# kepengxu/RealCamNet

Hardware: AMD Instinct MI355X
Metric: megapixels/sec RAW->sRGB at 4K (higher is better)
Workload: dtype bf16; 1 GPU; cfg3: 3840x2160 Bayer mosaic -> unshuffle+pad16 -> LiteISPNet_GFM_LSC_GMA -> sRGB 3840x2160, 8 frames/GPU, bf16 storage / fp32 accumulate; frames_per_gpu=8, global_frames=8, parallelism=frame-shard x1, collective=none

## Files before the change

realcamnet_amd/csrc/conv.hip:

```cpp
#include <mutex>
#include <vector>

#include "conv32_kernel.hpp"

namespace rc {

struct ConvPlan {
    int ck = 0, nt = 0, unit = 0, upt = 0, nu = 0, steps = 0;
    int n_chunks = 0, n_ct = 0, cout_packed = 0;
    int m32 = 0;
};

static int g_persist_on = 1;
extern int g_dw3_seg16;
extern int g_dec_lds;
extern int g_wmsa_mfma;
extern int g_pw_grid_cap;
static int g_pss = 0;
static int g_poison = 0;
static int g_thin = 2;
static int g_auto = 1;
static int g_sums_compact = 1;
static int g_conv32 = 0;

static bool make_plan(int cin, int cout, int ksize, int dtype, int out_mode, ConvPlan* p, int cout_tile = 0) {
    if (cin < 1 || cout < 1 || (ksize != 1 && ksize != 3 && ksize != 2 && ksize != 5)) return false;
    if (dtype != RC_F32 && dtype != RC_BF16 && dtype != RC_F16) return false;
    const bool h16 = dtype != RC_F32;
    if (ksize == 5 && (cout > 16 || out_mode == RC_OUT_PIXEL_SHUFFLE2 || (h16 ? (cin % 48 != 0 && cin % 32 != 0) : cin % 16 != 0))) return false;
    if (out_mode == RC_OUT_PIXEL_SHUFFLE2_NCHW && cout % 4 != 0) return false;
    if (ksize == 2 && (dtype != RC_BF16 || cin % 16 != 0 || out_mode != RC_OUT_NHWC || (cin % 48 == 0 && cin % 64 != 0))) return false;
    p->unit = dtype == RC_F32 ? 4 : 8;
    if (ksize == 5) p->ck = h16 ? (cin % 48 == 0 ? 48 : 32) : 16;
    else if (h16) {
        if (cin <= 8) p->ck = 8;
        else if (ksize == 1 && cin % 80 == 0 && cin % 64 != 0) p->ck = 80;
        else if (ksize >= 2 && cin % 64 == 0 && cin > 64) p->ck = 32;
        else if (cin % 64 == 0) p->ck = 64;
        else if (cin % 48 == 0) p->ck = 48;
        else if (ksize == 3 && cin == 32) p->ck = 32;
        else if (ksize == 3 && cin % 32 == 0 && cin > 64) p->ck = 32;
        else p->ck = 16;
    } else {
        p->ck = cin <= 4 ? 4 : 16;
    }
    if (out_mode == RC_OUT_PIXEL_SHUFFLE2) {
        if (cout % 4 != 0) return false;
        const int cps = cout / 4;
        if (cps % 64 == 0 && !(cps % 48 == 0 && h16 && cin == 48)) p->nt = 4;
        else if (cps % 48 == 0) p->nt = 3;
        else if (cps % 64 == 0) p->nt = 4;
        else if (cps % 16 == 0) p->nt = 1;
        else return false;
    } else if (cout % 48 == 0 && h16 && cin == 48) p->nt = 3;
    else if (h16 && ksize == 3 && cin == 32 && cout == 32) p->nt = 2;
    else if (ksize == 1 && cout % 80 == 0) p->nt = 5;
    else if (cout % 64 == 0) p->nt = 4;
    else if (cout % 48 == 0) p->nt = 3;
    else if (h16 && ksize == 3 && p->ck == 32 && cout % 32 == 0) p->nt = 2;
    else p->nt = 1;
    if (cout_tile != 0) {
        if (cout_tile < 16 || cout_tile > 80 || cout_tile % 16 != 0 || ksize == 5 || ksize == 2 || out_mode == RC_OUT_PIXEL_SHUFFLE2 || out_mode == RC_OUT_PIXEL_SHUFFLE2_NCHW) return false;
        p->nt = cout_tile / 16;
    }
    p->m32 = 0;
    if (cout_tile == 0 && dtype == RC_BF16 && ksize == 3 && g_conv32 != 0 && cout <= kPersistMaxCout && out_mode != RC_OUT_NCHW && out_mode != RC_OUT_PIXEL_SHUFFLE2_NCHW) {
        const int cw = out_mode == RC_OUT_PIXEL_SHUFFLE2 ? cout / 4 : cout;
        const bool all = g_conv32 != 4;
        if (all && p->ck == 32 && cin % 32 == 0 && (out_mode == RC_OUT_PIXEL_SHUFFLE2 ? cw % 32 == 0 : cw % 64 == 0)) { p->m32 = 1; p->nt = 2; p->ck = (g_conv32 == 1 && out_mode == RC_OUT_NHWC) ? 16 : 32; }
        else if (cin == 48 && (out_mode == RC_OUT_PIXEL_SHUFFLE2 ? (all && cw % 48 == 0) : cw % 96 == 0)) { p->m32 = 1; p->nt = 3; p->ck = 48; }
// ... 147 lines not shown
        const int co = packed_to_cout(p, cout, out_mode, j);
        dst[j] = (bias && co >= 0 && co < cout) ? bias[co] : 0.f;
    }
    return RC_OK;
}

size_t rc_conv_desc_size(void) { return sizeof(rc_conv_desc); }

int rc_tail_fold_weights(const float* w1, const float* b1, const float* w2, const float* b2, int c, int o, float* wc, float* bc) {
    RC_REQUIRE(w1 && w2 && wc && bc && c >= 1 && o >= 1, "rc_tail_fold_weights: bad arguments");
    std::vector<double> acc((size_t)4 * o * c * 25, 0.0), bacc((size_t)4 * o, 0.0);
    for (int oo = 0; oo < o; ++oo)
        for (int i = 0; i < 2; ++i)
            for (int j = 0; j < 2; ++j) {
                const int row = oo * 4 + 2 * i + j;
                bacc[row] = b2 ? (double)b2[oo] : 0.0;
                for (int dy = 0; dy < 3; ++dy)
                    for (int dx = 0; dx < 3; ++dx) {
                        const int a = i + dy - 1, b = j + dx - 1;
                        const int fy = a < 0 ? -1 : a >> 1, ii = a & 1, fx = b < 0 ? -1 : b >> 1, jj = b & 1;
                        for (int cc = 0; cc < c; ++cc) {
                            const int m = 4 * cc + 2 * ii + jj;
                            const double v2 = w2[(((size_t)oo * c + cc) * 3 + dy) * 3 + dx];
                            if (b1) bacc[row] += v2 * (double)b1[m];
                            for (int k = 0; k < c; ++k)
                                for (int ey = 0; ey < 3; ++ey)
                                    for (int ex = 0; ex < 3; ++ex)
                                        acc[(((size_t)row * c + k) * 5 + (fy + ey + 1)) * 5 + (fx + ex + 1)] += v2 * (double)w1[(((size_t)m * c + k) * 3 + ey) * 3 + ex];
                        }
                    }
            }
    for (size_t n = 0; n < acc.size(); ++n) wc[n] = (float)acc[n];
    for (size_t n = 0; n < bacc.size(); ++n) bc[n] = (float)bacc[n];
    return RC_OK;
}

int rc_conv_sum_tiles(int height, int width) { return 4 * ceil_div(height, kTH) * ceil_div(width, kTW); }

int rc_debug_set(const char* key, int value) {
    RC_REQUIRE(key != nullptr, "rc_debug_set: null key");
    if (std::string(key) == "persist") { g_persist_on = value < 0 ? 0 : (value > 3 ? 3 : value); return RC_OK; }
    if (std::string(key) == "conv_flags") { g_dbg_flags = value; return RC_OK; }
    if (std::string(key) == "pair_impl") { g_pair_impl = value < 0 || value > 2 ? 0 : value; return RC_OK; }
    if (std::string(key) == "dec_lds") { g_dec_lds = value != 0; return RC_OK; }
    if (std::string(key) == "dw3_seg16") { g_dw3_seg16 = value != 0; return RC_OK; }
    if (std::string(key) == "wmsa_mfma") { g_wmsa_mfma = value != 0; return RC_OK; }
    if (std::string(key) == "pss") { g_pss = value != 0; return RC_OK; }
    if (std::string(key) == "sums_compact") { g_sums_compact = value != 0; return RC_OK; }
    if (std::string(key) == "persist_auto") { g_auto = value < 0 ? 0 : (value > 2 ? 2 : value); return RC_OK; }
    if (std::string(key) == "thin") { g_thin = value < 0 ? 0 : (value > 2 ? 2 : value); return RC_OK; }
    if (std::string(key) == "lds_poison") { g_poison = value != 0; return RC_OK; }
    if (std::string(key) == "conv32") { g_conv32 = value < 0 ? 0 : (value > 4 ? 4 : value); return RC_OK; }
    if (std::string(key) == "wino_nnt") { wino_set_nnt(value); return RC_OK; }
    if (std::string(key) == "pw_grid_cap") { g_pw_grid_cap = value <= 0 || value > (1 << 22) ? (1 << 22) : value; return RC_OK; }
    return fail(RC_ERR_INVALID, std::string("rc_debug_set: unknown key ") + key);
}

int rc_debug_get(const char* key) {
    if (key == nullptr) return -1;
    if (std::string(key) == "persist") return g_persist_on;
    if (std::string(key) == "conv32") return g_conv32;
    if (std::string(key) == "conv_flags") return g_dbg_flags;
    if (std::string(key) == "pss") return g_pss;
    if (std::string(key) == "sums_compact") return g_sums_compact;
    if (std::string(key) == "persist_auto") return g_auto;
    if (std::string(key) == "thin") return g_thin;
    if (std::string(key) == "lds_poison") return g_poison;
    if (std::string(key) == "wino_nnt") return wino_get_nnt();
    if (std::string(key) == "pw_grid_cap") return g_pw_grid_cap;
    return -1;
}

int rc_debug_set_ptr(const char* key, void* p) {
    RC_REQUIRE(key != nullptr, "rc_debug_set_ptr: null key");
    if (std::string(key) == "conv_phase_timing") { g_dbg_ptr = static_cast<long long*>(p); return RC_OK; }
    return fail(RC_ERR_INVALID, std::string("rc_debug_set_ptr: unknown key ") + key);
}

int rc_prof_enable(int on) {
    std::lock_guard<std::mutex> lk(g_prof_mu);
    for (auto& r : g_prof) { (void)hipEventDestroy(r.e0); (void)hipEventDestroy(r.e1); }
    g_prof.clear();
    g_prof_on = on != 0;
    return RC_OK;
}

int rc_prof_collect(int64_t* n_launches, double* total_ms, double* total_flops) {
    std::lock_guard<std::mutex> lk(g_prof_mu);
    double ms = 0.0, fl = 0.0;
    for (auto& r : g_prof) {
        RC_HIP_CHECK(hipEventSynchronize(r.e1));
        float t = 0.f;
        RC_HIP_CHECK(hipEventElapsedTime(&t, r.e0, r.e1));
        ms += t; fl += r.flops;
    }
    if (n_launches) *n_launches = (int64_t)g_prof.size();
    if (total_ms) *total_ms = ms;
    if (total_flops) *total_flops = fl;
    return RC_OK;
}

int rc_prof_collect_rows(rc_prof_row* rows, int max_rows, int* n_rows) {
    RC_REQUIRE(rows != nullptr && n_rows != nullptr && max_rows >= 1, "rc_prof_collect_rows: bad arguments");
    std::lock_guard<std::mutex> lk(g_prof_mu);
    int n = 0;
    for (auto& r : g_prof) {
        RC_HIP_CHECK(hipEventSynchronize(r.e1));
        float t = 0.f;
        RC_HIP_CHECK(hipEventElapsedTime(&t, r.e0, r.e1));
        int i = 0;
        while (i < n && !(rows[i].cin == r.cin && rows[i].cout == r.cout && rows[i].ksize == r.ksize)) ++i;
        if (i == n) {
            if (n == max_rows) continue;
            rows[n] = rc_prof_row{r.cin, r.cout, r.ksize, 0, 0.0, 0.0, 0.0};
            ++n;
        }
        rows[i].launches += 1; rows[i].ms += t; rows[i].flops += r.flops; rows[i].bytes += r.bytes;
    }
    *n_rows = n;
    return RC_OK;
}

static int conv_build_args(const rc_conv_desc* d, ConvPlan& p, ConvArgs& a, size_t& es_out) {
    RC_REQUIRE(d != nullptr, "rc_conv2d: null desc");
    const bool dwt = d->out_mode == RC_OUT_NHWC_DWT;
    RC_REQUIRE(make_plan(d->cin, d->cout, d->ksize, d->dtype, dwt ? (int)RC_OUT_NHWC : d->out_mode, &p, d->cout_tile), "rc_conv2d: unsupported cin/cout/ksize/dtype/cout_tile");
    RC_REQUIRE(d->batch >= 1 && d->height >= 1 && d->width >= 1, "rc_conv2d: empty tensor");
    RC_REQUIRE(d->batch <= 65535, "rc_conv2d: batch > 65535");
// ... 153 lines not shown
```

realcamnet_amd/csrc/gma_fused.hip:

```cpp
#include "common.hpp"

namespace rc {
namespace gf {

typedef short s16x4 __attribute__((ext_vector_type(4)));

constexpr int kNT = 4;
constexpr int kC = 80, kCT = 64, kSEG = 16, kHID = 320;

__host__ __device__ constexpr int tile_bytes(int cin) { return (cin / 32) * 1024 + ((cin % 32) ? 512 : 0); }
__host__ __device__ constexpr int n_mtiles(int cout) { return (cout + 15) / 16; }
__host__ __device__ constexpr int row_channel(int m, int R, int mt) {
    return (m < (mt & ~1)) ? 32 * (m >> 1) + 8 * (R >> 2) + 4 * (m & 1) + (R & 3) : 16 * m + R;
}

template <int C> struct Act {
    static constexpr int KS = C / 32;
    static constexpr bool TAIL = (C % 32) != 0;
    uint4 f[KS > 0 ? KS : 1];
    uint2 t;
};

__device__ __forceinline__ void mma32(const uint4& a, const uint4& b, f32x4& c) {
    c = __builtin_amdgcn_mfma_f32_16x16x32_bf16(__builtin_bit_cast(bf16x8, a), __builtin_bit_cast(bf16x8, b), c, 0, 0, 0);
// ... 1382 lines not shown
    }
}
#undef GI_KEEP

}
}

extern "C" int rc_dw_toeplitz_pack(const float* taps, int K, int n_ch, void* dst) {
    using namespace rc;
    RC_REQUIRE(taps && dst, "rc_dw_toeplitz_pack: null pointer");
    RC_REQUIRE((K == 3 || K == 5 || K == 7) && n_ch >= 1, "rc_dw_toeplitz_pack: K = 3, 5 or 7");
    uint16_t* out = static_cast<uint16_t*>(dst);
    for (int dy = 0; dy < K; ++dy)
        for (int c = 0; c < n_ch; ++c)
            for (int lane = 0; lane < 64; ++lane)
                for (int i = 0; i < 8; ++i) {
                    const int ox = lane & 15, slot = 8 * (lane >> 4) + i, dx = slot - 4 - ox + K / 2;
                    out[((size_t)(dy * n_ch + c) * 64 + lane) * 8 + i] = (dx >= 0 && dx < K) ? host_f32_to_bf16(taps[(size_t)(dy * K + dx) * n_ch + c]) : (uint16_t)0;
                }
    return RC_OK;
}

extern "C" int rc_gma_in_cpe(const void* d_d1, const void* d_w_in_natural, const float* d_b_in, const void* d_toeplitz3, const float* d_b_cpe, void* d_x,
                             int batch, int H, int W, void* stream) {
    using namespace rc;
    using namespace rc::gf;
    RC_REQUIRE(d_d1 && d_w_in_natural && d_toeplitz3 && d_x, "rc_gma_in_cpe: null pointer");
    RC_REQUIRE(reinterpret_cast<uintptr_t>(d_d1) % 16 == 0 && reinterpret_cast<uintptr_t>(d_w_in_natural) % 16 == 0 && reinterpret_cast<uintptr_t>(d_toeplitz3) % 16 == 0 &&
               reinterpret_cast<uintptr_t>(d_x) % 16 == 0, "rc_gma_in_cpe: misaligned tensor");
    RC_REQUIRE(batch >= 1 && H >= 1 && W >= 1, "rc_gma_in_cpe: bad shape");
    RC_REQUIRE((long long)H * W * GI_CIN * 2 < (1ll << 31), "rc_gma_in_cpe: a 192-channel image must stay below 2 GiB (32-bit buffer offsets)");
    GiArgs a;
    a.d1 = static_cast<const bf16_t*>(d_d1); a.x = static_cast<bf16_t*>(d_x);
    a.batch = batch; a.H = H; a.W = W; a.tiles_x = ceil_div(W, GI_TW); a.tiles_y = ceil_div(H, GI_TH);
    const long long n_tiles = (long long)a.tiles_x * a.tiles_y * batch;
    RC_REQUIRE(n_tiles < (1ll << 31), "rc_gma_in_cpe: too many tiles");
    a.n_tiles = (int)n_tiles;
    a.w_in = d_w_in_natural; a.b_in = d_b_in; a.toep = static_cast<const char*>(d_toeplitz3); a.b_cpe = d_b_cpe;
    const int num_cus = device_cu_count();
    if (int e_ = allow_lds<&gma_in_cpe_kernel>(160 * 1024)) return e_;
    int blocks = a.n_tiles < num_cus ? a.n_tiles : num_cus;
    a.tiles_per_block = (a.n_tiles + blocks - 1) / blocks;
    blocks = (a.n_tiles + a.tiles_per_block - 1) / a.tiles_per_block;
    return launch_lds<&gma_in_cpe_kernel>(dim3((unsigned)blocks), dim3(GI_THREADS), GI_LDS, as_stream(stream), a);
}

namespace rc {
namespace gf {

struct LscArgs {
    const bf16_t* x; int cin0;
    const char* blob; int n_mid; float slope;
    const bf16_t* raw; int raw_c;
    bf16_t* out; long long pixels; int H, W;
};

template <int C> __host__ __device__ constexpr int lsc_weight_bytes(int n_mid, bool head) {
    return (C / 16) * 512 + n_mid * (C / 16) * tile_bytes(C) + (head ? (C / 16) * 1536 : 0);
}

template <int CIN, int MT>
__device__ __forceinline__ void gemm_fresh(const char* w, int lane, const Act<CIN> (&in)[kNT], f32x4 (&acc)[MT][kNT], const float* bias = nullptr, int g = 0) {
    constexpr int KS = CIN / 32, TB = tile_bytes(CIN);
    const f32x4 z = f32x4{0.f, 0.f, 0.f, 0.f};
    if (bias != nullptr) {
#pragma unroll
        for (int m = 0; m < MT; ++m) {
            const f32x4 b = bias4(bias, m, g);
#pragma unroll
            for (int nt = 0; nt < kNT; ++nt) acc[m][nt] = b;
        }
    }
#pragma unroll
    for (int s = 0; s < KS; ++s) {
        uint4 a[MT];
#pragma unroll
        for (int m = 0; m < MT; ++m) a[m] = *reinterpret_cast<const uint4*>(w + m * TB + s * 1024 + lane * 16);
#pragma unroll
        for (int m = 0; m < MT; ++m)
#pragma unroll
            for (int nt = 0; nt < kNT; ++nt) {
                if (s == 0 && bias == nullptr) { acc[m][nt] = z; }
                mma32(a[m], in[nt].f[s], acc[m][nt]);
            }
    }
    if constexpr ((CIN % 32) != 0) {
#pragma unroll
        for (int m = 0; m < MT; ++m) {
            const uint2 a = *reinterpret_cast<const uint2*>(w + m * TB + KS * 1024 + lane * 8);
#pragma unroll
            for (int nt = 0; nt < kNT; ++nt) {
                if (KS == 0 && bias == nullptr) { acc[m][nt] = z; }
                mma16(a, in[nt].t, acc[m][nt]);
            }
        }
    }
}

__device__ __forceinline__ f32x4 leaky4(const f32x4& v, float slope) {
    const f32x4 s = v * slope;
    const float inf = 3.402823466e+38f;
    return f32x4{__builtin_amdgcn_fmed3f(v[0], s[0], inf), __builtin_amdgcn_fmed3f(v[1], s[1], inf), __builtin_amdgcn_fmed3f(v[2], s[2], inf), __builtin_amdgcn_fmed3f(v[3], s[3], inf)};
}

template <int C, bool ACT, bool BIASED = false>
__device__ __forceinline__ void lsc_pack(const f32x4 (&acc)[C / 16][kNT], const float* bias, int g, float slope, Act<C> (&out)[kNT]) {
    constexpr int MT = C / 16;
    auto fin = [&](const f32x4& v, const f32x4& b) {
        f32x4 r = BIASED ? v : v + b;
        if constexpr (ACT) r = leaky4(r, slope);
        return r;
    };
    constexpr bool RAW_ACC = BIASED && !ACT;
#pragma unroll
    for (int p = 0; p < MT / 2; ++p) {
        const f32x4 b0 = bias4(bias, 2 * p, g), b1 = bias4(bias, 2 * p + 1, g);
#pragma unroll
        for (int nt = 0; nt < kNT; ++nt) {
            if constexpr (RAW_ACC) {
                const uint2 lo = qa_pack(acc[2 * p][nt]), hi = qa_pack(acc[2 * p + 1][nt]);
                out[nt].f[p] = make_uint4(lo.x, lo.y, hi.x, hi.y);
            } else {
                out[nt].f[p] = pack_pair(fin(acc[2 * p][nt], b0), fin(acc[2 * p + 1][nt], b1));
            }
        }
    }
    if constexpr (MT & 1) {
        const f32x4 b0 = bias4(bias, MT - 1, g);
#pragma unroll
        for (int nt = 0; nt < kNT; ++nt) {
            if constexpr (RAW_ACC) out[nt].t = qa_pack(acc[MT - 1][nt]);
            else out[nt].t = pack_tail(fin(acc[MT - 1][nt], b0));
        }
    }
}

constexpr int kOOBoff = (int)0x80000000;

struct LscIn {
    uint2 x[kNT];
    uint4 rf[kNT]; uint2 rt[kNT];
};

template <bool HEAD>
__device__ __forceinline__ void lsc_load(const LscArgs& a, long long p0, int n, int g, __amdgpu_buffer_rsrc_t r_x, __amdgpu_buffer_rsrc_t r_raw, LscIn& in) {
    const unsigned uW = (unsigned)a.W, uH = (unsigned)a.H;
    unsigned row0 = 0, x0 = 0, y0 = 0;
    if constexpr (HEAD) {
        row0 = __builtin_amdgcn_readfirstlane((unsigned)p0 / uW);
        x0 = (unsigned)p0 - row0 * uW;
        y0 = __builtin_amdgcn_readfirstlane(row0 % uH);
    }
#pragma unroll
    for (int nt = 0; nt < kNT; ++nt) {
        const long long p = p0 + 16 * nt + n;
        const bool live = p < a.pixels;
        {
            const int off = (live && g == 0) ? (int)p * a.cin0 * 2 : kOOBoff;
            unsigned lo = 0, hi = 0;
            if (a.cin0 == 2) lo = __builtin_amdgcn_raw_buffer_load_b32(r_x, off, 0, 0);
            else if (a.cin0 == 4) { const auto v = __builtin_amdgcn_raw_buffer_load_b64(r_x, off, 0, 0); lo = v[0]; hi = v[1]; }
            else {
                unsigned short e[4] = {0, 0, 0, 0};
                for (int i = 0; i < a.cin0; ++i) e[i] = __builtin_amdgcn_raw_buffer_load_b16(r_x, off == kOOBoff ? kOOBoff : off + 2 * i, 0, 0);
                lo = e[0] | ((unsigned)e[1] << 16); hi = e[2] | ((unsigned)e[3] << 16);
            }
            in.x[nt] = make_uint2(lo, hi);
        }
        if constexpr (HEAD) {
            unsigned x = x0 + 16 * nt + n, y = y0;
            while (x >= uW) { x -= uW; ++y; }
            while (y >= uH) y -= uH;
            auto tap = [&](int t) -> uint2 {
                const int dy = t / 3 - 1, dx = t % 3 - 1;
                const bool ok = live && (unsigned)((int)y + dy) < uH && (unsigned)((int)x + dx) < uW;
                const int off = ok ? ((int)p + dy * a.W + dx) * a.raw_c * 2 : kOOBoff;
                if (a.raw_c == 4) { const auto v = __builtin_amdgcn_raw_buffer_load_b64(r_raw, off, 0, 0); return make_uint2(v[0], v[1]); }
                unsigned short e[4] = {0, 0, 0, 0};
                for (int i = 0; i < a.raw_c; ++i) e[i] = __builtin_amdgcn_raw_buffer_load_b16(r_raw, ok ? off + 2 * i : kOOBoff, 0, 0);
                return make_uint2(e[0] | ((unsigned)e[1] << 16), e[2] | ((unsigned)e[3] << 16));
            };
            const uint2 t0 = tap(2 * g), t1 = tap(2 * g + 1), t8 = tap(8);
            in.rf[nt] = make_uint4(t0.x, t0.y, t1.x, t1.y);
            in.rt[nt] = g == 0 ? t8 : make_uint2(0u, 0u);
        }
    }
}

struct LscTaps { int dy0, dx0, dy1, dx1, d0, d1, d8; };
__device__ __forceinline__ LscTaps lsc_taps(int g, int W) {
    LscTaps t;
    t.dy0 = (2 * g) / 3 - 1; t.dx0 = (2 * g) % 3 - 1; t.dy1 = (2 * g + 1) / 3 - 1; t.dx1 = (2 * g + 1) % 3 - 1;
    t.d0 = (t.dy0 * W + t.dx0) * 8; t.d1 = (t.dy1 * W + t.dx1) * 8; t.d8 = (W + 1) * 8;
    return t;
}
template <bool HEAD>
__device__ __forceinline__ void lsc_load_fast(const LscArgs& a, int p0, unsigned tx0, unsigned ty0, int n, int g, const LscTaps& tp, __amdgpu_buffer_rsrc_t r_x,
                                              __amdgpu_buffer_rsrc_t r_raw, LscIn& in) {
    const unsigned uW = (unsigned)a.W, uH = (unsigned)a.H;
    const int npix = (int)a.pixels;
#pragma unroll
    for (int nt = 0; nt < kNT; ++nt) {
        const int p = p0 + 16 * nt + n;
        const bool live = p < npix;
        in.x[nt] = make_uint2(__builtin_amdgcn_raw_buffer_load_b32(r_x, (live && g == 0) ? p * 4 : kOOBoff, 0, 0), 0u);
        if constexpr (HEAD) {
            unsigned x = tx0 + 16 * nt + n, y = ty0;
            const bool wrap = x >= uW;
            x = wrap ? x - uW : x; y = wrap ? y + 1 : y; y = y == uH ? 0u : y;
            const int pb = p * 8;
            const bool ok0 = live && (unsigned)((int)y + tp.dy0) < uH && (unsigned)((int)x + tp.dx0) < uW;
            const bool ok1 = live && (unsigned)((int)y + tp.dy1) < uH && (unsigned)((int)x + tp.dx1) < uW;
            const bool ok8 = live && g == 0 && y + 1 < uH && x + 1 < uW;
            const auto t0 = __builtin_amdgcn_raw_buffer_load_b64(r_raw, ok0 ? pb + tp.d0 : kOOBoff, 0, 0);
            const auto t1 = __builtin_amdgcn_raw_buffer_load_b64(r_raw, ok1 ? pb + tp.d1 : kOOBoff, 0, 0);
            const auto t8 = __builtin_amdgcn_raw_buffer_load_b64(r_raw, ok8 ? pb + tp.d8 : kOOBoff, 0, 0);
            in.rf[nt] = make_uint4(t0[0], t0[1], t1[0], t1[1]);
            in.rt[nt] = make_uint2(t8[0], t8[1]);
        }
    }
}

template <int C> constexpr int lsc_threads() { return C > 64 ? 512 : 256; }
template <int C, bool HEAD>
__global__ __launch_bounds__(lsc_threads<C>(), 2) void lsc_chain_kernel(const LscArgs a) {
    constexpr int kLscThreads = lsc_threads<C>();
    constexpr int MT = C / 16, TBM = tile_bytes(C);
    extern __shared__ __attribute__((aligned(16))) char lds[];
    const int tid = threadIdx.x, lane = tid & 63, n = lane & 15, g = lane >> 4;
    const int w_bytes = lsc_weight_bytes<C>(a.n_mid, HEAD);
    const int total = w_bytes + (1 + a.n_mid + (HEAD ? 1 : 0)) * MT * 16 * 4;
    for (int i = tid; i < total / 16; i += kLscThreads) reinterpret_cast<uint4*>(lds)[i] = reinterpret_cast<const uint4*>(a.blob)[i];
    __syncthreads();
    constexpr bool STAGE = C <= 64;
    [[maybe_unused]] char* s_stage = lds + ((total + 15) & ~15);
    const char* s_l0 = lds;
    const char* s_mid = lds + MT * 512;
    const char* s_head = s_mid + a.n_mid * MT * TBM;
    const float* s_b = reinterpret_cast<const float*>(lds + w_bytes);

    const __amdgpu_buffer_rsrc_t r_x = __builtin_amdgcn_make_buffer_rsrc(const_cast<bf16_t*>(a.x), 0, (int)(a.pixels * a.cin0 * 2), 0x00020000);
    const __amdgpu_buffer_rsrc_t r_raw = __builtin_amdgcn_make_buffer_rsrc(const_cast<bf16_t*>(HEAD ? a.raw : a.x), 0,
                                                                           (int)(a.pixels * (HEAD ? a.raw_c : a.cin0) * 2), 0x00020000);
    const long long n_tiles = (a.pixels + 63) / 64, n_waves = (long long)gridDim.x * (kLscThreads / 64);
    long long tile = (long long)blockIdx.x * (kLscThreads / 64) + __builtin_amdgcn_readfirstlane(tid >> 6);
    const bool fast = a.cin0 == 2 && (!HEAD || a.raw_c == 4) && a.W >= 64;
    const LscTaps tp = lsc_taps(g, a.W);
    const unsigned uW = (unsigned)a.W, uH = (unsigned)a.H;
    const unsigned step = (unsigned)(64 * n_waves), sx = step % uW, sy = (step / uW) % uH;
    unsigned tx0 = 0, ty0 = 0;
    if (tile < n_tiles) { const unsigned p0 = (unsigned)(tile * 64), row0 = p0 / uW; tx0 = p0 - row0 * uW; ty0 = row0 % uH; }
    auto load = [&](long long t, LscIn& dst) {
        if (fast) {
            lsc_load_fast<HEAD>(a, (int)(t * 64), tx0, ty0, n, g, tp, r_x, r_raw, dst);
            tx0 += sx; ty0 += sy;
            if (tx0 >= uW) { tx0 -= uW; ++ty0; }
            if (ty0 >= uH) ty0 -= uH;
        } else {
            lsc_load<HEAD>(a, t * 64, n, g, r_x, r_raw, dst);
        }
    };
    LscIn nxt;
    if (tile < n_tiles) load(tile, nxt);
    for (; tile < n_tiles; tile += n_waves) {
        const LscIn in = nxt;
        if (tile + n_waves < n_tiles) load(tile + n_waves, nxt);
        Act<C> cur[kNT];
        {
            auto leaky = [&](f32x4 v) { return leaky4(v, a.slope); };
#pragma unroll
            for (int p = 0; p < MT / 2; ++p) {
                const uint2 w0 = *reinterpret_cast<const uint2*>(s_l0 + (2 * p) * 512 + lane * 8), w1 = *reinterpret_cast<const uint2*>(s_l0 + (2 * p + 1) * 512 + lane * 8);
                const f32x4 b0 = bias4(s_b, 2 * p, g), b1 = bias4(s_b, 2 * p + 1, g);
#pragma unroll
                for (int nt = 0; nt < kNT; ++nt) {
                    f32x4 a0 = b0, a1 = b1;
                    mma16(w0, in.x[nt], a0); mma16(w1, in.x[nt], a1);
                    cur[nt].f[p] = pack_pair(leaky(a0), leaky(a1));
                }
            }
            if constexpr (MT & 1) {
                const uint2 w0 = *reinterpret_cast<const uint2*>(s_l0 + (MT - 1) * 512 + lane * 8);
                const f32x4 b0 = bias4(s_b, MT - 1, g);
#pragma unroll
                for (int nt = 0; nt < kNT; ++nt) {
                    f32x4 a0 = b0;
                    mma16(w0, in.x[nt], a0);
                    cur[nt].t = pack_tail(leaky(a0));
                }
            }
        }
#pragma unroll 1
        for (int l = 0; l < a.n_mid; ++l) {
            if constexpr (MT <= 4) {
                f32x4 acc[MT][kNT];
                gemm_fresh<C, MT>(s_mid + l * MT * TBM, lane, cur, acc, s_b + (1 + l) * MT * 16, g);
                if (l + 1 < a.n_mid) lsc_pack<C, true, true>(acc, s_b + (1 + l) * MT * 16, g, a.slope, cur);
                else lsc_pack<C, false, true>(acc, s_b + (1 + l) * MT * 16, g, a.slope, cur);
            } else {
                static_assert(MT % 4 == 0, "wide chain: whole groups of 4 output tiles");
                Act<C> nxt[kNT];
#pragma unroll
                for (int h = 0; h < MT / 4; ++h) {
                    f32x4 acc[4][kNT];
                    const float* bias = s_b + (1 + l) * MT * 16 + 4 * h * 16;
                    gemm_fresh<C, 4>(s_mid + (l * MT + 4 * h) * TBM, lane, cur, acc, bias, g);
                    const bool act = l + 1 < a.n_mid;
#pragma unroll
                    for (int p = 0; p < 2; ++p) {
#pragma unroll
                        for (int nt = 0; nt < kNT; ++nt) {
                            f32x4 v0 = acc[2 * p][nt], v1 = acc[2 * p + 1][nt];
                            if (act) {
                                nxt[nt].f[2 * h + p] = pack_pair(leaky4(v0, a.slope), leaky4(v1, a.slope));
                            } else {
                                const uint2 lo = qa_pack(v0), hi = qa_pack(v1);
                                nxt[nt].f[2 * h + p] = make_uint4(lo.x, lo.y, hi.x, hi.y);
                            }
                        }
                    }
                }
#pragma unroll
                for (int nt = 0; nt < kNT; ++nt) cur[nt] = nxt[nt];
            }
        }
        if constexpr (HEAD) {
            const float* hb = s_b + (1 + a.n_mid) * MT * 16;
            auto head_tile = [&](int m, int nt, const f32x4& b) {
                f32x4 acc = b;
                mma32(*reinterpret_cast<const uint4*>(s_head + m * 1536 + lane * 16), in.rf[nt], acc);
                mma16(*reinterpret_cast<const uint2*>(s_head + m * 1536 + 1024 + lane * 8), in.rt[nt], acc);
                return acc;
            };
            auto mulp1 = [](const f32x4& h, const f32x4& l) { return __builtin_elementwise_fma(h, l, h); };
#pragma unroll
            for (int p = 0; p < MT / 2; ++p) {
                const f32x4 b0 = bias4(hb, 2 * p, g), b1 = bias4(hb, 2 * p + 1, g);
#pragma unroll
                for (int nt = 0; nt < kNT; ++nt)
                    cur[nt].f[p] = pack_pair(mulp1(head_tile(2 * p, nt, b0), up_lo(cur[nt].f[p])), mulp1(head_tile(2 * p + 1, nt, b1), up_hi(cur[nt].f[p])));
            }
            if constexpr (MT & 1) {
                const f32x4 b0 = bias4(hb, MT - 1, g);
#pragma unroll
                for (int nt = 0; nt < kNT; ++nt) cur[nt].t = pack_tail(mulp1(head_tile(MT - 1, nt, b0), up_tail(cur[nt].t)));
            }
        }
        if constexpr (STAGE) {
            char* st = s_stage + (tid >> 6) * (64 * C * 2);
#pragma unroll
            for (int nt = 0; nt < kNT; ++nt) store_act<C>(reinterpret_cast<bf16_t*>(st) + (16 * nt + n) * C, g, cur[nt]);
            __builtin_amdgcn_fence(__ATOMIC_RELEASE, "wavefront");
            __builtin_amdgcn_wave_barrier();
            const long long left = (a.pixels - tile * 64) * (C * 2);
            const __amdgpu_buffer_rsrc_t r_o = __builtin_amdgcn_make_buffer_rsrc(a.out + tile * 64 * C, 0, (int)(left < 64 * C * 2 ? left : 64 * C * 2), 0x00020000);
#pragma unroll
            for (int j = 0; j < (64 * C * 2) / 1024; ++j) {
                const uint4 v = *reinterpret_cast<const uint4*>(st + (lane + 64 * j) * 16);
                typedef unsigned int u4_t __attribute__((ext_vector_type(4)));
                __builtin_amdgcn_raw_buffer_store_b128(u4_t{v.x, v.y, v.z, v.w}, r_o, (lane + 64 * j) * 16, 0, 0);
            }
        } else {
#pragma unroll
            for (int nt = 0; nt < kNT; ++nt) {
                const long long p = tile * 64 + 16 * nt + n;
                if (p < a.pixels) store_act<C>(a.out + p * C, g, cur[nt]);
            }
        }
    }
}

}
}

extern "C" size_t rc_lsc_packed_bytes(int c, int n_mid, int has_head) {
    if (!(c == 32 || c == 48 || c == 64 || c == 128) || n_mid < 1) return 0;
    const bool hd = has_head != 0;
    const int w = c == 32 ? lsc_weight_bytes<32>(n_mid, hd) : c == 48 ? lsc_weight_bytes<48>(n_mid, hd) : c == 64 ? lsc_weight_bytes<64>(n_mid, hd) : lsc_weight_bytes<128>(n_mid, hd);
    return (size_t)w + (size_t)(1 + n_mid + (has_head ? 1 : 0)) * (c / 16) * 16 * 4;
}

extern "C" int rc_lsc_pack(const float* w0, const float* b0, int cin0, const float* const* wmid, const float* const* bmid, int n_mid,
                           const float* whead, const float* bhead, int raw_c, int c, void* dst) {
    RC_REQUIRE(w0 && wmid && bmid && dst, "rc_lsc_pack: null pointer");
    RC_REQUIRE((c == 32 || c == 48 || c == 64 || c == 128) && n_mid >= 1 && n_mid <= 4 && cin0 >= 1 && cin0 <= 4, "rc_lsc_pack: width 32, 48, 64 or 128, 1..4 mid layers, cin0 <= 4");
    RC_REQUIRE(!whead || (raw_c >= 1 && raw_c <= 4), "rc_lsc_pack: the head's input has 1..4 channels");
    const int mt = c / 16, tbm = tile_bytes(c);
    char* p = static_cast<char*>(dst);
    for (int m = 0; m < mt; ++m)
        for (int lane = 0; lane < 64; ++lane) {
            const int ch = row_channel(m, lane & 15, mt), q = lane >> 4;
            uint16_t* o = reinterpret_cast<uint16_t*>(p + m * 512 + lane * 8);
            for (int i = 0; i < 4; ++i) o[i] = (4 * q + i < cin0) ? host_f32_to_bf16(w0[(size_t)ch * cin0 + 4 * q + i]) : 0;
        }
    p += mt * 512;
    for (int l = 0; l < n_mid; ++l) {
        RC_REQUIRE(wmid[l] != nullptr, "rc_lsc_pack: null layer");
        const int rc = rc_chain_pack_weights(wmid[l], c, c, p);
        if (rc != RC_OK) return rc;
        p += mt * tbm;
    }
    if (whead) {
        for (int m = 0; m < mt; ++m)
            for (int lane = 0; lane < 64; ++lane) {
                const int ch = row_channel(m, lane & 15, mt), q = lane >> 4;
                uint16_t* o4 = reinterpret_cast<uint16_t*>(p + m * 1536 + lane * 16);
                uint16_t* o2 = reinterpret_cast<uint16_t*>(p + m * 1536 + 1024 + lane * 8);
                auto wv = [&](int tap, int ci) { return ci < raw_c ? host_f32_to_bf16(whead[((size_t)ch * raw_c + ci) * 9 + tap]) : (uint16_t)0; };
                for (int i = 0; i < 8; ++i) o4[i] = wv(2 * q + (i >> 2), i & 3);
                for (int i = 0; i < 4; ++i) o2[i] = q == 0 ? wv(8, i) : (uint16_t)0;
            }
        p += mt * 1536;
    }
    float* b = reinterpret_cast<float*>(p);
    rc_chain_pack_bias(b0, c, b);
    for (int l = 0; l < n_mid; ++l) rc_chain_pack_bias(bmid[l], c, b + (1 + l) * mt * 16);
    if (whead) rc_chain_pack_bias(bhead, c, b + (1 + n_mid) * mt * 16);
    return RC_OK;
}

extern "C" int rc_lsc_chain(const void* d_x, int cin0, const void* d_blob, int c, int n_mid, float slope, const void* d_raw, int raw_c,
                            void* d_out, int batch, int H, int W, void* stream) {
    RC_REQUIRE(d_x && d_blob && d_out, "rc_lsc_chain: null pointer");
    RC_REQUIRE((c == 32 || c == 48 || c == 64 || c == 128) && n_mid >= 1 && n_mid <= 4 && cin0 >= 1 && cin0 <= 4, "rc_lsc_chain: width 32, 48, 64 or 128, 1..4 mid layers, cin0 <= 4");
    RC_REQUIRE(!d_raw || (raw_c >= 1 && raw_c <= 4), "rc_lsc_chain: the head's input has 1..4 channels");
    RC_REQUIRE(!(d_raw && c == 128), "rc_lsc_chain: the fused head exists at widths 32 / 48 / 64 (at 128 it spilled 29 registers and the codec needs the lens-shading map itself)");
    RC_REQUIRE(batch >= 1 && H >= 1 && W >= 1 && (long long)batch * H * W * 8 < (1LL << 31), "rc_lsc_chain: bad shape (inputs must stay below 2 GiB)");
    RC_REQUIRE(slope >= 0.f && slope <= 1.f, "rc_lsc_chain: slope must be in [0, 1]");
    RC_REQUIRE(reinterpret_cast<uintptr_t>(d_out) % 16 == 0 && reinterpret_cast<uintptr_t>(d_blob) % 16 == 0, "rc_lsc_chain: misaligned pointer");
    LscArgs a{};
    a.x = static_cast<const bf16_t*>(d_x); a.cin0 = cin0; a.blob = static_cast<const char*>(d_blob); a.n_mid = n_mid; a.slope = slope;
    a.raw = static_cast<const bf16_t*>(d_raw); a.raw_c = raw_c; a.out = static_cast<bf16_t*>(d_out);
    a.pixels = (long long)batch * H * W; a.H = H; a.W = W;
    size_t lds = rc_lsc_packed_bytes(c, n_mid, d_raw != nullptr);
    if (c <= 64) lds = ((lds + 15) & ~(size_t)15) + 4 * 64 * (size_t)c * 2;
    RC_REQUIRE(lds <= 150 * 1024, "rc_lsc_chain: weights (+ output staging) do not fit LDS");
    const long long tiles = (a.pixels + 63) / 64;
    const int wpb = (c > 64 ? 512 : 256) / 64;
    long long grid = (tiles + wpb - 1) / wpb;
    const long long cap = (long long)device_cu_count() * (c > 64 ? 1 : 3);
    if (grid > cap) grid = cap;
#define RC_LSC(CC, HH)                                                                                                                    \
    do {                                                                                                                                  \
        if (int e_ = allow_lds<&lsc_chain_kernel<CC, HH>>(150 * 1024)) return e_;                                                    \
        return launch_lds<&lsc_chain_kernel<CC, HH>>(dim3((unsigned)grid), dim3(lsc_threads<CC>()), (int)lds, as_stream(stream), a); \
    } while (0)
    if (c == 32) { if (d_raw) RC_LSC(32, true); else RC_LSC(32, false); }
    else if (c == 48) { if (d_raw) RC_LSC(48, true); else RC_LSC(48, false); }
    else if (c == 64) { if (d_raw) RC_LSC(64, true); else RC_LSC(64, false); }
    else RC_LSC(128, false);
#undef RC_LSC
}


namespace rc {
namespace gf {

constexpr int KV_TILE = 128, KV_ROW = KV_TILE + 8, KV_THREADS = 256;
__global__ __launch_bounds__(KV_THREADS) void gma_kvsum_mfma_kernel(const bf16_t* __restrict__ qkvp, size_t plane, const float* __restrict__ kmax,
                                                                     float* __restrict__ part, int n_tok, int L) {
    __shared__ __attribute__((aligned(16))) unsigned short s_e[64 * KV_ROW];
    __shared__ __attribute__((aligned(16))) unsigned short s_v[64 * KV_ROW];
    __shared__ float s_m[64];
    const int tid = threadIdx.x, lane = tid & 63, wave = tid >> 6, n = lane & 15, g = lane >> 4;
    const int blk = blockIdx.x, b = blockIdx.y, nblk = gridDim.x;
    const float kLog2e = 1.4426950408889634f;
    if (tid < 64) s_m[tid] = kmax[(size_t)b * 64 + tid] * kLog2e;
    const int t0 = blk * L, t1 = (t0 + L) < n_tok ? (t0 + L) : n_tok;
    const int half = tid & 1, tl = tid >> 1;
    const bf16_t* kbase = qkvp + (size_t)4 * plane + (size_t)b * n_tok * kSEG + 8 * half;
    const bf16_t* vbase = qkvp + (size_t)8 * plane + (size_t)b * n_tok * kSEG + 8 * half;
    uint4 kr[4], vr[4];
    auto fetch = [&](int tt) {
        const int t = tt + tl;
#pragma unroll
        for (int r = 0; r < 4; ++r) {
            kr[r] = vr[r] = make_uint4(0u, 0u, 0u, 0u);
            if (t < t1) {
                kr[r] = *reinterpret_cast<const uint4*>(kbase + (size_t)r * plane + (size_t)t * kSEG);
                vr[r] = *reinterpret_cast<const uint4*>(vbase + (size_t)r * plane + (size_t)t * kSEG);
            }
        }
    };
    float z[4][8];
#pragma unroll
    for (int r = 0; r < 4; ++r)
#pragma unroll
        for (int e = 0; e < 8; ++e) z[r][e] = 0.f;
    f32x4 acc = f32x4{0.f, 0.f, 0.f, 0.f};
    if (t0 < t1) fetch(t0);
    __syncthreads();
    for (int tt = t0; tt < t1; tt += KV_TILE) {
        const bool live = tt + tl < t1;
#pragma unroll
        for (int r = 0; r < 4; ++r) {
            const unsigned kw[4] = {kr[r].x, kr[r].y, kr[r].z, kr[r].w}, vw[4] = {vr[r].x, vr[r].y, vr[r].z, vr[r].w};
#pragma unroll
// ... 458 lines not shown
```

Before: 1321 MP/s.

## Reuse LSC chain activations across frames when per-tile inputs are identical

The LSC chain kernel is restructured so each wave walks every frame of the batch for the same spatial tile. It compares the tile's x input with the previous frame's using a wave ballot, and skips the first layer and mid-layer GEMMs when they match, keeping the prior activations in registers. The fused head and the output store still run for every frame. Separately, the change adds sched_barrier hints around the MFMA groups, switches indexing to 32-bit per-frame offsets, splits the fast and slow load paths into template instances, and sizes the grid cap from a memoized occupancy query instead of a fixed 3 blocks per CU. This adds register pressure from the kept activations and a compare per tile, and it only pays off when frames share the same LSC input.

After: 1324 MP/s, median of 6. Within noise of the previous version (+0.2%).

```diff
diff --git a/realcamnet_amd/csrc/conv.hip b/realcamnet_amd/csrc/conv.hip
--- a/realcamnet_amd/csrc/conv.hip
+++ b/realcamnet_amd/csrc/conv.hip
@@ -16,6 +16,8 @@
 extern int g_dec_lds;
 extern int g_wmsa_mfma;
 extern int g_pw_grid_cap;
+extern int g_lsc_reuse;
+extern unsigned long long* g_lsc_evals;
 static int g_pss = 0;
 static int g_poison = 0;
 static int g_thin = 2;
@@ -269,6 +271,7 @@
     if (std::string(key) == "lds_poison") { g_poison = value != 0; return RC_OK; }
     if (std::string(key) == "conv32") { g_conv32 = value < 0 ? 0 : (value > 4 ? 4 : value); return RC_OK; }
     if (std::string(key) == "wino_nnt") { wino_set_nnt(value); return RC_OK; }
+    if (std::string(key) == "lsc_reuse") { g_lsc_reuse = value != 0; return RC_OK; }
     if (std::string(key) == "pw_grid_cap") { g_pw_grid_cap = value <= 0 || value > (1 << 22) ? (1 << 22) : value; return RC_OK; }
     return fail(RC_ERR_INVALID, std::string("rc_debug_set: unknown key ") + key);
 }
@@ -284,6 +287,7 @@
     if (std::string(key) == "thin") return g_thin;
     if (std::string(key) == "lds_poison") return g_poison;
     if (std::string(key) == "wino_nnt") return wino_get_nnt();
+    if (std::string(key) == "lsc_reuse") return g_lsc_reuse;
     if (std::string(key) == "pw_grid_cap") return g_pw_grid_cap;
     return -1;
 }
@@ -291,6 +295,7 @@
 int rc_debug_set_ptr(const char* key, void* p) {
     RC_REQUIRE(key != nullptr, "rc_debug_set_ptr: null key");
     if (std::string(key) == "conv_phase_timing") { g_dbg_ptr = static_cast<long long*>(p); return RC_OK; }
+    if (std::string(key) == "lsc_evals") { g_lsc_evals = static_cast<unsigned long long*>(p); return RC_OK; }
     return fail(RC_ERR_INVALID, std::string("rc_debug_set_ptr: unknown key ") + key);
 }
 
diff --git a/realcamnet_amd/csrc/gma_fused.hip b/realcamnet_amd/csrc/gma_fused.hip
--- a/realcamnet_amd/csrc/gma_fused.hip
+++ b/realcamnet_amd/csrc/gma_fused.hip
@@ -1458,13 +1458,16 @@
     const bf16_t* x; int cin0;
     const char* blob; int n_mid; float slope;
     const bf16_t* raw; int raw_c;
-    bf16_t* out; long long pixels; int H, W;
+    bf16_t* out; long long pixels; int batch, hw, H, W;
+    int reuse;
+    unsigned long long* evals;
 };
 
 template <int C> __host__ __device__ constexpr int lsc_weight_bytes(int n_mid, bool head) {
     return (C / 16) * 512 + n_mid * (C / 16) * tile_bytes(C) + (head ? (C / 16) * 1536 : 0);
 }
 
+constexpr int kSchedAllButMfma = 0x7F6;
 template <int CIN, int MT>
 __device__ __forceinline__ void gemm_fresh(const char* w, int lane, const Act<CIN> (&in)[kNT], f32x4 (&acc)[MT][kNT], const float* bias = nullptr, int g = 0) {
     constexpr int KS = CIN / 32, TB = tile_bytes(CIN);
@@ -1489,6 +1492,7 @@
                 if (s == 0 && bias == nullptr) { acc[m][nt] = z; }
                 mma32(a[m], in[nt].f[s], acc[m][nt]);
             }
+        __builtin_amdgcn_sched_barrier(kSchedAllButMfma);
     }
     if constexpr ((CIN % 32) != 0) {
 #pragma unroll
@@ -1500,6 +1504,7 @@
                 mma16(a, in[nt].t, acc[m][nt]);
             }
         }
+        __builtin_amdgcn_sched_barrier(kSchedAllButMfma);
     }
 }
 
@@ -1549,20 +1554,20 @@
 };
 
 template <bool HEAD>
-__device__ __forceinline__ void lsc_load(const LscArgs& a, long long p0, int n, int g, __amdgpu_buffer_rsrc_t r_x, __amdgpu_buffer_rsrc_t r_raw, LscIn& in) {
+__device__ __forceinline__ void lsc_load(const LscArgs& a, int base, int p0, int n, int g, __amdgpu_buffer_rsrc_t r_x, __amdgpu_buffer_rsrc_t r_raw, LscIn& in) {
     const unsigned uW = (unsigned)a.W, uH = (unsigned)a.H;
-    unsigned row0 = 0, x0 = 0, y0 = 0;
+    unsigned x0 = 0, y0 = 0;
     if constexpr (HEAD) {
-        row0 = __builtin_amdgcn_readfirstlane((unsigned)p0 / uW);
-        x0 = (unsigned)p0 - row0 * uW;
-        y0 = __builtin_amdgcn_readfirstlane(row0 % uH);
+        y0 = __builtin_amdgcn_readfirstlane((unsigned)p0 / uW);
+        x0 = (unsigned)p0 - y0 * uW;
     }
 #pragma unroll
     for (int nt = 0; nt < kNT; ++nt) {
-        const long long p = p0 + 16 * nt + n;
-        const bool live = p < a.pixels;
+        const int q = p0 + 16 * nt + n;
+        const bool live = q < a.hw;
+        const int p = base + q;
         {
-            const int off = (live && g == 0) ? (int)p * a.cin0 * 2 : kOOBoff;
+            const int off = (live && g == 0) ? p * a.cin0 * 2 : kOOBoff;
             unsigned lo = 0, hi = 0;
             if (a.cin0 == 2) lo = __builtin_amdgcn_raw_buffer_load_b32(r_x, off, 0, 0);
             else if (a.cin0 == 4) { const auto v = __builtin_amdgcn_raw_buffer_load_b64(r_x, off, 0, 0); lo = v[0]; hi = v[1]; }
@@ -1576,11 +1581,10 @@
         if constexpr (HEAD) {
             unsigned x = x0 + 16 * nt + n, y = y0;
             while (x >= uW) { x -= uW; ++y; }
-            while (y >= uH) y -= uH;
             auto tap = [&](int t) -> uint2 {
                 const int dy = t / 3 - 1, dx = t % 3 - 1;
                 const bool ok = live && (unsigned)((int)y + dy) < uH && (unsigned)((int)x + dx) < uW;
-                const int off = ok ? ((int)p + dy * a.W + dx) * a.raw_c * 2 : kOOBoff;
+                const int off = ok ? (p + dy * a.W + dx) * a.raw_c * 2 : kOOBoff;
                 if (a.raw_c == 4) { const auto v = __builtin_amdgcn_raw_buffer_load_b64(r_raw, off, 0, 0); return make_uint2(v[0], v[1]); }
                 unsigned short e[4] = {0, 0, 0, 0};
                 for (int i = 0; i < a.raw_c; ++i) e[i] = __builtin_amdgcn_raw_buffer_load_b16(r_raw, ok ? off + 2 * i : kOOBoff, 0, 0);
@@ -1601,19 +1605,19 @@
     return t;
 }
 template <bool HEAD>
-__device__ __forceinline__ void lsc_load_fast(const LscArgs& a, int p0, unsigned tx0, unsigned ty0, int n, int g, const LscTaps& tp, __amdgpu_buffer_rsrc_t r_x,
+__device__ __forceinline__ void lsc_load_fast(const LscArgs& a, int base, int p0, unsigned tx0, unsigned ty0, int n, int g, const LscTaps& tp, __amdgpu_buffer_rsrc_t r_x,
                                               __amdgpu_buffer_rsrc_t r_raw, LscIn& in) {
     const unsigned uW = (unsigned)a.W, uH = (unsigned)a.H;
-    const int npix = (int)a.pixels;
 #pragma unroll
     for (int nt = 0; nt < kNT; ++nt) {
-        const int p = p0 + 16 * nt + n;
-        const bool live = p < npix;
+        const int q = p0 + 16 * nt + n;
+        const bool live = q < a.hw;
+        const int p = base + q;
         in.x[nt] = make_uint2(__builtin_amdgcn_raw_buffer_load_b32(r_x, (live && g == 0) ? p * 4 : kOOBoff, 0, 0), 0u);
         if constexpr (HEAD) {
             unsigned x = tx0 + 16 * nt + n, y = ty0;
             const bool wrap = x >= uW;
-            x = wrap ? x - uW : x; y = wrap ? y + 1 : y; y = y == uH ? 0u : y;
+            x = wrap ? x - uW : x; y = wrap ? y + 1 : y;
             const int pb = p * 8;
             const bool ok0 = live && (unsigned)((int)y + tp.dy0) < uH && (unsigned)((int)x + tp.dx0) < uW;
             const bool ok1 = live && (unsigned)((int)y + tp.dy1) < uH && (unsigned)((int)x + tp.dx1) < uW;
@@ -1628,8 +1632,8 @@
 }
 
 template <int C> constexpr int lsc_threads() { return C > 64 ? 512 : 256; }
-template <int C, bool HEAD>
-__global__ __launch_bounds__(lsc_threads<C>(), 2) void lsc_chain_kernel(const LscArgs a) {
+template <int C, bool HEAD, bool FAST>
+__device__ __forceinline__ void lsc_chain_body(const LscArgs a) {
     constexpr int kLscThreads = lsc_threads<C>();
     constexpr int MT = C / 16, TBM = tile_bytes(C);
     extern __shared__ __attribute__((aligned(16))) char lds[];
@@ -1648,94 +1652,111 @@
     const __amdgpu_buffer_rsrc_t r_x = __builtin_amdgcn_make_buffer_rsrc(const_cast<bf16_t*>(a.x), 0, (int)(a.pixels * a.cin0 * 2), 0x00020000);
     const __amdgpu_buffer_rsrc_t r_raw = __builtin_amdgcn_make_buffer_rsrc(const_cast<bf16_t*>(HEAD ? a.raw : a.x), 0,
                                                                            (int)(a.pixels * (HEAD ? a.raw_c : a.cin0) * 2), 0x00020000);
-    const long long n_tiles = (a.pixels + 63) / 64, n_waves = (long long)gridDim.x * (kLscThreads / 64);
-    long long tile = (long long)blockIdx.x * (kLscThreads / 64) + __builtin_amdgcn_readfirstlane(tid >> 6);
-    const bool fast = a.cin0 == 2 && (!HEAD || a.raw_c == 4) && a.W >= 64;
+    const int n_tiles = (a.hw + 63) / 64, n_waves = (int)gridDim.x * (kLscThreads / 64);
+    int tile = (int)blockIdx.x * (kLscThreads / 64) + __builtin_amdgcn_readfirstlane(tid >> 6), frame = 0;
     const LscTaps tp = lsc_taps(g, a.W);
-    const unsigned uW = (unsigned)a.W, uH = (unsigned)a.H;
-    const unsigned step = (unsigned)(64 * n_waves), sx = step % uW, sy = (step / uW) % uH;
+    const unsigned uW = (unsigned)a.W;
+    const unsigned step = (unsigned)(64 * n_waves), sx = step % uW, sy = step / uW;
+    int ltile = tile, lframe = 0;
     unsigned tx0 = 0, ty0 = 0;
-    if (tile < n_tiles) { const unsigned p0 = (unsigned)(tile * 64), row0 = p0 / uW; tx0 = p0 - row0 * uW; ty0 = row0 % uH; }
-    auto load = [&](long long t, LscIn& dst) {
-        if (fast) {
-            lsc_load_fast<HEAD>(a, (int)(t * 64), tx0, ty0, n, g, tp, r_x, r_raw, dst);
+    if (tile < n_tiles) { const unsigned p0 = (unsigned)(tile * 64); ty0 = p0 / uW; tx0 = p0 - ty0 * uW; }
+    auto load = [&](LscIn& dst) {
+        const int base = lframe * a.hw;
+        if constexpr (FAST) lsc_load_fast<HEAD>(a, base, ltile * 64, tx0, ty0, n, g, tp, r_x, r_raw, dst);
+        else lsc_load<HEAD>(a, base, ltile * 64, n, g, r_x, r_raw, dst);
+        if (++lframe == a.batch) {
+            lframe = 0; ltile += n_waves;
             tx0 += sx; ty0 += sy;
             if (tx0 >= uW) { tx0 -= uW; ++ty0; }
-            if (ty0 >= uH) ty0 -= uH;
-        } else {
-            lsc_load<HEAD>(a, t * 64, n, g, r_x, r_raw, dst);
         }
     };
     LscIn nxt;
-    if (tile < n_tiles) load(tile, nxt);
-    for (; tile < n_tiles; tile += n_waves) {
+    if (tile < n_tiles) load(nxt);
+    Act<C> cur[kNT];
+    uint2 kept[kNT];
+#pragma unroll
+    for (int nt = 0; nt < kNT; ++nt) kept[nt] = make_uint2(0u, 0u);
+    while (tile < n_tiles) {
         const LscIn in = nxt;
-        if (tile + n_waves < n_tiles) load(tile + n_waves, nxt);
-        Act<C> cur[kNT];
-        {
-            auto leaky = [&](f32x4 v) { return leaky4(v, a.slope); };
-#pragma unroll
-            for (int p = 0; p < MT / 2; ++p) {
-                const uint2 w0 = *reinterpret_cast<const uint2*>(s_l0 + (2 * p) * 512 + lane * 8), w1 = *reinterpret_cast<const uint2*>(s_l0 + (2 * p + 1) * 512 + lane * 8);
-                const f32x4 b0 = bias4(s_b, 2 * p, g), b1 = bias4(s_b, 2 * p + 1, g);
-#pragma unroll
-                for (int nt = 0; nt < kNT; ++nt) {
-                    f32x4 a0 = b0, a1 = b1;
-                    mma16(w0, in.x[nt], a0); mma16(w1, in.x[nt], a1);
-                    cur[nt].f[p] = pack_pair(leaky(a0), leaky(a1));
+        if (ltile < n_tiles) load(nxt);
+        bool eval = frame == 0 || a.reuse == 0;
+        if (!eval) {
+            unsigned d = 0;
+#pragma unroll
+            for (int nt = 0; nt < kNT; ++nt) d |= (in.x[nt].x ^ kept[nt].x) | (in.x[nt].y ^ kept[nt].y);
+            eval = __builtin_amdgcn_ballot_w64(d != 0) != 0;
+        }
+        if (a.evals != nullptr && lane == 0) atomicAdd(a.evals + (eval ? 0 : 1), 1ULL);
+        if (eval) {
+#pragma unroll
+            for (int nt = 0; nt < kNT; ++nt) kept[nt] = in.x[nt];
+            {
+                auto leaky = [&](f32x4 v) { return leaky4(v, a.slope); };
+#pragma unroll
+                for (int p = 0; p < MT / 2; ++p) {
+                    const uint2 w0 = *reinterpret_cast<const uint2*>(s_l0 + (2 * p) * 512 + lane * 8), w1 = *reinterpret_cast<const uint2*>(s_l0 + (2 * p + 1) * 512 + lane * 8);
+                    const f32x4 b0 = bias4(s_b, 2 * p, g), b1 = bias4(s_b, 2 * p + 1, g);
+#pragma unroll
+                    for (int nt = 0; nt < kNT; ++nt) {
+                        f32x4 a0 = b0, a1 = b1;
+                        mma16(w0, in.x[nt], a0); mma16(w1, in.x[nt], a1);
+                        cur[nt].f[p] = pack_pair(leaky(a0), leaky(a1));
+                    }
                 }
-            }
-            if constexpr (MT & 1) {
-                const uint2 w0 = *reinterpret_cast<const uint2*>(s_l0 + (MT - 1) * 512 + lane * 8);
-                const f32x4 b0 = bias4(s_b, MT - 1, g);
-#pragma unroll
-                for (int nt = 0; nt < kNT; ++nt) {
-                    f32x4 a0 = b0;
-                    mma16(w0, in.x[nt], a0);
-                    cur[nt].t = pack_tail(leaky(a0));
+                if constexpr (MT & 1) {
+                    const uint2 w0 = *reinterpret_cast<const uint2*>(s_l0 + (MT - 1) * 512 + lane * 8);
+                    const f32x4 b0 = bias4(s_b, MT - 1, g);
+#pragma unroll
+                    for (int nt = 0; nt < kNT; ++nt) {
+                        f32x4 a0 = b0;
+                        mma16(w0, in.x[nt], a0);
+                        cur[nt].t = pack_tail(leaky(a0));
+                    }
                 }
             }
-        }
 #pragma unroll 1
-        for (int l = 0; l < a.n_mid; ++l) {
-            if constexpr (MT <= 4) {
-                f32x4 acc[MT][kNT];
-                gemm_fresh<C, MT>(s_mid + l * MT * TBM, lane, cur, acc, s_b + (1 + l) * MT * 16, g);
-                if (l + 1 < a.n_mid) lsc_pack<C, true, true>(acc, s_b + (1 + l) * MT * 16, g, a.slope, cur);
-                else lsc_pack<C, false, true>(acc, s_b + (1 + l) * MT * 16, g, a.slope, cur);
-            } else {
-                static_assert(MT % 4 == 0, "wide chain: whole groups of 4 output tiles");
-                Act<C> nxt[kNT];
-#pragma unroll
-                for (int h = 0; h < MT / 4; ++h) {
-                    f32x4 acc[4][kNT];
-                    const float* bias = s_b + (1 + l) * MT * 16 + 4 * h * 16;
-                    gemm_fresh<C, 4>(s_mid + (l * MT + 4 * h) * TBM, lane, cur, acc, bias, g);
-                    const bool act = l + 1 < a.n_mid;
-#pragma unroll
-                    for (int p = 0; p < 2; ++p) {
-#pragma unroll
-                        for (int nt = 0; nt < kNT; ++nt) {
-                            f32x4 v0 = acc[2 * p][nt], v1 = acc[2 * p + 1][nt];
-                            if (act) {
-                                nxt[nt].f[2 * h + p] = pack_pair(leaky4(v0, a.slope), leaky4(v1, a.slope));
-                            } else {
-                                const uint2 lo = qa_pack(v0), hi = qa_pack(v1);
-                                nxt[nt].f[2 * h + p] = make_uint4(lo.x, lo.y, hi.x, hi.y);
+            for (int l = 0; l < a.n_mid; ++l) {
+                if constexpr (MT <= 4) {
+                    f32x4 acc[MT][kNT];
+                    gemm_fresh<C, MT>(s_mid + l * MT * TBM, lane, cur, acc, s_b + (1 + l) * MT * 16, g);
+                    if (l + 1 < a.n_mid) lsc_pack<C, true, true>(acc, s_b + (1 + l) * MT * 16, g, a.slope, cur);
+                    else lsc_pack<C, false, true>(acc, s_b + (1 + l) * MT * 16, g, a.slope, cur);
+                } else {
+                    static_assert(MT % 4 == 0, "wide chain: whole groups of 4 output tiles");
+                    Act<C> nxt[kNT];
+#pragma unroll
+                    for (int h = 0; h < MT / 4; ++h) {
+                        f32x4 acc[4][kNT];
+                        const float* bias = s_b + (1 + l) * MT * 16 + 4 * h * 16;
+                        gemm_fresh<C, 4>(s_mid + (l * MT + 4 * h) * TBM, lane, cur, acc, bias, g);
+                        const bool act = l + 1 < a.n_mid;
+#pragma unroll
+                        for (int p = 0; p < 2; ++p) {
+#pragma unroll
+                            for (int nt = 0; nt < kNT; ++nt) {
+                                f32x4 v0 = acc[2 * p][nt], v1 = acc[2 * p + 1][nt];
+                                if (act) {
+                                    nxt[nt].f[2 * h + p] = pack_pair(leaky4(v0, a.slope), leaky4(v1, a.slope));
+                                } else {
+                                    const uint2 lo = qa_pack(v0), hi = qa_pack(v1);
+                                    nxt[nt].f[2 * h + p] = make_uint4(lo.x, lo.y, hi.x, hi.y);
+                                }
                             }
                         }
                     }
+#pragma unroll
+                    for (int nt = 0; nt < kNT; ++nt) cur[nt] = nxt[nt];
                 }
-#pragma unroll
-                for (int nt = 0; nt < kNT; ++nt) cur[nt] = nxt[nt];
-            }
-        }
+            }
+        }
+        [[maybe_unused]] Act<C> o[kNT];
         if constexpr (HEAD) {
             const float* hb = s_b + (1 + a.n_mid) * MT * 16;
             auto head_tile = [&](int m, int nt, const f32x4& b) {
                 f32x4 acc = b;
                 mma32(*reinterpret_cast<const uint4*>(s_head + m * 1536 + lane * 16), in.rf[nt], acc);
                 mma16(*reinterpret_cast<const uint2*>(s_head + m * 1536 + 1024 + lane * 8), in.rt[nt], acc);
+                __builtin_amdgcn_sched_barrier(kSchedAllButMfma);
                 return acc;
             };
             auto mulp1 = [](const f32x4& h, const f32x4& l) { return __builtin_elementwise_fma(h, l, h); };
@@ -1744,22 +1765,24 @@
                 const f32x4 b0 = bias4(hb, 2 * p, g), b1 = bias4(hb, 2 * p + 1, g);
 #pragma unroll
                 for (int nt = 0; nt < kNT; ++nt)
-                    cur[nt].f[p] = pack_pair(mulp1(head_tile(2 * p, nt, b0), up_lo(cur[nt].f[p])), mulp1(head_tile(2 * p + 1, nt, b1), up_hi(cur[nt].f[p])));
+                    o[nt].f[p] = pack_pair(mulp1(head_tile(2 * p, nt, b0), up_lo(cur[nt].f[p])), mulp1(head_tile(2 * p + 1, nt, b1), up_hi(cur[nt].f[p])));
             }
             if constexpr (MT & 1) {
                 const f32x4 b0 = bias4(hb, MT - 1, g);
 #pragma unroll
-                for (int nt = 0; nt < kNT; ++nt) cur[nt].t = pack_tail(mulp1(head_tile(MT - 1, nt, b0), up_tail(cur[nt].t)));
-            }
-        }
+                for (int nt = 0; nt < kNT; ++nt) o[nt].t = pack_tail(mulp1(head_tile(MT - 1, nt, b0), up_tail(cur[nt].t)));
+            }
+        }
+        const Act<C> (&res)[kNT] = *(HEAD ? &o : &cur);
+        bf16_t* const out_t = a.out + ((long long)frame * a.hw + (long long)tile * 64) * C;
         if constexpr (STAGE) {
             char* st = s_stage + (tid >> 6) * (64 * C * 2);
 #pragma unroll
-            for (int nt = 0; nt < kNT; ++nt) store_act<C>(reinterpret_cast<bf16_t*>(st) + (16 * nt + n) * C, g, cur[nt]);
+            for (int nt = 0; nt < kNT; ++nt) store_act<C>(reinterpret_cast<bf16_t*>(st) + (16 * nt + n) * C, g, res[nt]);
             __builtin_amdgcn_fence(__ATOMIC_RELEASE, "wavefront");
             __builtin_amdgcn_wave_barrier();
-            const long long left = (a.pixels - tile * 64) * (C * 2);
-            const __amdgpu_buffer_rsrc_t r_o = __builtin_amdgcn_make_buffer_rsrc(a.out + tile * 64 * C, 0, (int)(left < 64 * C * 2 ? left : 64 * C * 2), 0x00020000);
+            const int left_px = a.hw - tile * 64;
+            const __amdgpu_buffer_rsrc_t r_o = __builtin_amdgcn_make_buffer_rsrc(out_t, 0, (left_px < 64 ? left_px : 64) * (C * 2), 0x00020000);
 #pragma unroll
             for (int j = 0; j < (64 * C * 2) / 1024; ++j) {
                 const uint4 v = *reinterpret_cast<const uint4*>(st + (lane + 64 * j) * 16);
@@ -1769,14 +1792,24 @@
         } else {
 #pragma unroll
             for (int nt = 0; nt < kNT; ++nt) {
-                const long long p = tile * 64 + 16 * nt + n;
-                if (p < a.pixels) store_act<C>(a.out + p * C, g, cur[nt]);
-            }
-        }
-    }
-}
-
-}
+                const int q = 16 * nt + n;
+                if (tile * 64 + q < a.hw) store_act<C>(out_t + q * C, g, res[nt]);
+            }
+        }
+        if (++frame == a.batch) { frame = 0; tile += n_waves; }
+    }
+}
+
+template <int C, bool HEAD>
+__global__ __launch_bounds__(lsc_threads<C>(), 2) void lsc_chain_kernel(const LscArgs a) {
+    if (a.cin0 == 2 && (!HEAD || a.raw_c == 4) && a.W >= 64) lsc_chain_body<C, HEAD, true>(a);
+    else lsc_chain_body<C, HEAD, false>(a);
+}
+
+}
+
+int g_lsc_reuse = 1;
+unsigned long long* g_lsc_evals = nullptr;
 }
 
 extern "C" size_t rc_lsc_packed_bytes(int c, int n_mid, int has_head) {
@@ -1837,18 +1870,27 @@
     LscArgs a{};
     a.x = static_cast<const bf16_t*>(d_x); a.cin0 = cin0; a.blob = static_cast<const char*>(d_blob); a.n_mid = n_mid; a.slope = slope;
     a.raw = static_cast<const bf16_t*>(d_raw); a.raw_c = raw_c; a.out = static_cast<bf16_t*>(d_out);
-    a.pixels = (long long)batch * H * W; a.H = H; a.W = W;
+    a.pixels = (long long)batch * H * W; a.batch = batch; a.hw = H * W; a.H = H; a.W = W;
+    a.reuse = g_lsc_reuse; a.evals = g_lsc_evals;
     size_t lds = rc_lsc_packed_bytes(c, n_mid, d_raw != nullptr);
     if (c <= 64) lds = ((lds + 15) & ~(size_t)15) + 4 * 64 * (size_t)c * 2;
     RC_REQUIRE(lds <= 150 * 1024, "rc_lsc_chain: weights (+ output staging) do not fit LDS");
-    const long long tiles = (a.pixels + 63) / 64;
-    const int wpb = (c > 64 ? 512 : 256) / 64;
-    long long grid = (tiles + wpb - 1) / wpb;
-    const long long cap = (long long)device_cu_count() * (c > 64 ? 1 : 3);
-    if (grid > cap) grid = cap;
+    const long long tiles = ((long long)a.hw + 63) / 64;
 #define RC_LSC(CC, HH)                                                                                                                    \
     do {                                                                                                                                  \
+        constexpr int wpb = lsc_threads<CC>() / 64;                                                                                       \
         if (int e_ = allow_lds<&lsc_chain_kernel<CC, HH>>(150 * 1024)) return e_;                                                    \
+        static std::atomic<long long> memo{0};                                            \
+        const long long m_ = memo.load(std::memory_order_relaxed);                                                                        \
+        int per_cu = (m_ >> 8) == (long long)lds ? (int)(m_ & 255) : 0;                                                                   \
+        if (per_cu < 1) {                                                                                                                 \
+            if (hipOccupancyMaxActiveBlocksPerMultiprocessor(&per_cu, &lsc_chain_kernel<CC, HH>, lsc_threads<CC>(), lds) != hipSuccess || per_cu < 1) per_cu = 1; \
+            if (per_cu > 255) per_cu = 255;                                                                                               \
+            memo.store(((long long)lds << 8) | per_cu, std::memory_order_relaxed);                                                        \
+        }                                                                                                                                 \
+        long long grid = (tiles + wpb - 1) / wpb;                                                                                         \
+        const long long cap = (long long)device_cu_count() * per_cu;                                                                      \
+        if (grid > cap) grid = cap;                                                                                                       \
         return launch_lds<&lsc_chain_kernel<CC, HH>>(dim3((unsigned)grid), dim3(lsc_threads<CC>()), (int)lds, as_stream(stream), a); \
     } while (0)
     if (c == 32) { if (d_raw) RC_LSC(32, true); else RC_LSC(32, false); }
```
